# vt-asaplab/porla

Measured on NVIDIA B200. Metric: G1 MSM points/sec, higher is better.
Workload: dtype u32 (8x32-bit limb Montgomery, IMAD carry chains)

## Files before the change

### porla_b200/csrc/affine_kernels.cuh

```cuda
#pragma once
#include "msm_kernels.cuh"

namespace porla {

constexpr int kAffL = 64;
constexpr int kAffCap1 = 44;
constexpr int kAffCap2 = 24;
constexpr int kAffMaxAdds = 32;
constexpr int kAffThreads = 128;
constexpr int kAffDefaultRounds = 0;
#ifndef PORLA_AFF_MIN_BLOCKS
#define PORLA_AFF_MIN_BLOCKS 3
#endif

enum : uint32_t { kOpCopy = 0, kOpAdd = 1, kOpDbl = 2, kOpInf = 3 };

template <class C>
struct AffSrc {
    using F = typename C::F;
    const Affine<F>* points;
    const F* phi_x;
    uint32_t phi_off;
    const uint2* pairs;
    const Affine<F>* arr;
    const uint32_t* keys;

    PORLA_D uint32_t key(int i) const { return pairs ? __ldg(&pairs[i].x) : keys[i]; }
    PORLA_D Affine<F> pt(int i) const {
        if (pairs) return load_signed_point<C>(points, phi_x, phi_off, __ldg(&pairs[i].y));
        return arr[i];
    }
    PORLA_D F ptx(int i) const {
        if (pairs) {
            const uint32_t idx = __ldg(&pairs[i].y) & 0x7fffffffu;
            const bool image = C::kGlv && phi_off != 0 && idx >= phi_off;
            const uint32_t j = image ? idx - phi_off : idx;
            const uint4* sx = image ? reinterpret_cast<const uint4*>(phi_x + j) : reinterpret_cast<const uint4*>(points + j);
            F x;
            uint4* d = reinterpret_cast<uint4*>(&x);
            d[0] = __ldg(sx);
            d[1] = __ldg(sx + 1);
            return x;
        }
        return arr[i].x;
    }
};

template <class C>
PORLA_D int aff_count_outputs(const AffSrc<C>& src, int n) {
    int outs = 0, i = 0;
    while (i < n) {
        const uint32_t k = src.key(i);
        i += (i + 1 < n && src.key(i + 1) == k) ? 2 : 1;
        outs++;
    }
    return outs;
}

template <class C>
PORLA_D int aff_round(const AffSrc<C>& src, int n, uint64_t in_inf, Affine<typename C::F>* out, uint32_t* out_keys,
                      typename C::F* pre, uint8_t* opi, uint64_t* out_inf) {
    using F = typename C::F;
    int i = 0, j = 0, na = 0;
    F acc = F::one();
    while (i < n) {
        const uint32_t k = src.key(i);
        const bool pair = i + 1 < n && src.key(i + 1) == k;
        uint32_t type = kOpCopy, idx = (uint32_t)i;
        if (pair) {
            const bool inf0 = (in_inf >> i) & 1u, inf1 = (in_inf >> (i + 1)) & 1u;
            if (inf0 || inf1) {
                if (inf0 && inf1) type = kOpInf;
                else idx = (uint32_t)(inf0 ? i + 1 : i);
            } else {
                F den = src.ptx(i + 1) - src.ptx(i);
                type = kOpAdd;
                if (den.is_zero()) {
                    const Affine<F> p = src.pt(i), q = src.pt(i + 1);
                    if (p.y == q.y && !p.y.is_zero()) {
                        den = p.y.dbl();
                        type = kOpDbl;
                    } else {
                        type = kOpInf;
                    }
                }
                if (type != kOpInf) {
                    pre[na++] = acc;
                    acc = acc * den;
                }
            }
        } else if ((in_inf >> i) & 1u) {
            type = kOpInf;
        }
        opi[j] = (uint8_t)(idx | (type << 6));
        out_keys[j] = k;
        i += pair ? 2 : 1;
        j++;
    }
    const int outs = j;
    F inv = F::one();
    if (na > 0) inv = acc.inverse();
    uint64_t infm = 0;
    for (j = outs - 1; j >= 0; j--) {
        const uint32_t idx = opi[j] & 63u, type = opi[j] >> 6;
        if (type == kOpCopy) {
            out[j] = src.pt((int)idx);
        } else if (type == kOpInf) {
            infm |= 1ull << j;
        } else {
            const Affine<F> p = src.pt((int)idx), q = src.pt((int)idx + 1);
            const F den = type == kOpAdd ? q.x - p.x : p.y.dbl();
            const F inv_j = inv * pre[--na];
            inv = inv * den;
            F lam, x3;
            if (type == kOpAdd) {
                lam = (q.y - p.y) * inv_j;
                x3 = lam.sqr() - p.x - q.x;
            } else {
                const F xx = p.x.sqr();
                lam = (xx.dbl() + xx) * inv_j;
                x3 = lam.sqr() - p.x.dbl();
            }
            Affine<F> r;
            r.x = x3;
            r.y = lam * (p.x - x3) - p.y;
            out[j] = r;
        }
    }
    *out_inf = infm;
    return outs;
}

template <class C>
__global__ void __launch_bounds__(kAffThreads, PORLA_AFF_MIN_BLOCKS)
k_accumulate_affine(const Affine<typename C::F>* __restrict__ points, const typename C::F* __restrict__ phi_x, uint32_t phi_off,
                    const uint2* __restrict__ sorted, const uint32_t* __restrict__ total_pairs,
                    XYZZ<typename C::F>* __restrict__ buckets, XYZZ<typename C::F>* __restrict__ part_head,
                    XYZZ<typename C::F>* __restrict__ part_tail, int rounds) {
    using F = typename C::F;
    const uint32_t M = *total_pairs;
    const uint32_t t = blockIdx.x * blockDim.x + threadIdx.x;
    const uint64_t start64 = (uint64_t)t * kAffL;
    if (start64 >= M) return;
    const uint32_t start = (uint32_t)start64;
    const uint32_t end = (M - start > (uint32_t)kAffL) ? start + kAffL : M;
    const uint32_t prev_key = start > 0 ? __ldg(&sorted[start - 1].x) : 0xffffffffu;
    const uint32_t next_key = end < M ? __ldg(&sorted[end].x) : 0xffffffffu;

    Affine<F> p1[kAffCap1], p2[kAffCap2];
    F pre[kAffMaxAdds];
    uint32_t k1[kAffCap1], k2[kAffCap2];
    uint8_t opi[kAffCap1];

    AffSrc<C> cur;
    cur.points = points;
    cur.phi_x = phi_x;
    cur.phi_off = phi_off;
    cur.pairs = sorted + start;
    cur.arr = nullptr;
    cur.keys = nullptr;
    int n = (int)(end - start);
    uint64_t inf = 0;

    if (rounds >= 1) {
        const int outs0 = aff_count_outputs<C>(cur, n);
        if (outs0 <= kAffCap1 && outs0 < n) {
            n = aff_round<C>(cur, n, inf, p1, k1, pre, opi, &inf);
            cur.pairs = nullptr;
            cur.arr = p1;
            cur.keys = k1;
            if (rounds >= 2) {
                const int outs1 = aff_count_outputs<C>(cur, n);
                if (outs1 <= kAffCap2 && outs1 < n) {
                    n = aff_round<C>(cur, n, inf, p2, k2, pre, opi, &inf);
                    cur.arr = p2;
                    cur.keys = k2;
                }
            }
        }
    }

    int i = 0;
    while (i < n) {
        const uint32_t key = cur.key(i);
        const bool first_run = i == 0;
        XYZZ<F> acc = XYZZ<F>::inf();
        if (!((inf >> i) & 1u)) {
            const Affine<F> p = cur.pt(i);
            acc = XYZZ<F>{p.x, p.y, F::one(), F::one()};
        }
        i++;
        while (i < n && cur.key(i) == key) {
            if (!((inf >> i) & 1u)) acc.madd(cur.pt(i));
            i++;
        }
        const bool last_run = i == n;
        if (first_run && prev_key == key) st16(part_head + t, acc);
        else if (last_run && next_key == key) st16(part_tail + t, acc);
        else st16(buckets + key, acc);
    }
}

}
```

### porla_b200/csrc/msm_impl.cuh

```cuda
#pragma once
#include <atomic>
#include <cstdio>
#include <cstdlib>
#include <mutex>
#include <type_traits>

#include "arena.h"
#include "msm.h"
#include "msm_kernels.cuh"
#include "small_kernels.cuh"
#include "affine_kernels.cuh"

namespace porla {

extern std::atomic<uint64_t> g_launches;
#define LAUNCHED() (g_launches.fetch_add(1, std::memory_order_relaxed))



template <class C> struct CurveIdOf;
template <> struct CurveIdOf<Bn254> { static constexpr int value = kCurveBn254; };
template <> struct CurveIdOf<Secp256k1> { static constexpr int value = kCurveSecp256k1; };

template <class C>
// ... 161 lines not shown
    sh.c = wplan.c;
    sh.nwin = glv ? 2 * wplan.nwin : (C::kScalarBits + 1 + sh.c - 1) / sh.c;
    int slice_shift = 0;
    while ((1 << slice_shift) < opt.slice_count) slice_shift++;
    if (opt.slice_count > 1) {
        const bool ok = (1 << slice_shift) == opt.slice_count && opt.slice_index >= 0 && opt.slice_index < opt.slice_count &&
                        !fixed && nbatch == 1 && opt.window_bits > 0 && opt.glv >= 0 && opt.no_fixed_base &&
                        msm_max_slices(wplan, opt.slice_count) == opt.slice_count;
        if (!ok) {
            fprintf(stderr, "[libmultiexp/porla_b200] FATAL: bucket slice %d of %d: needs one MSM, a forced window layout and a power-of-two "
                            "slice count that leaves whole coarse bins (c = %d)\n", opt.slice_index, opt.slice_count, wplan.c);
            abort();
        }
    }
    sh.slice_shift = (uint32_t)slice_shift;
    sh.slice_r = opt.slice_count > 1 ? (uint32_t)opt.slice_index : 0u;
    sh.nbuckets = (1u << (sh.c - 1)) >> slice_shift;
    sh.fixed_n = fixed ? table.fb_n : 0u;
    sh.glv_wh = glv ? wplan.nwin : 0;
    sh.phi_off = glv ? table.phi_off : 0u;
    const int slot_windows = fixed ? 1 : (glv ? wplan.nwin : sh.nwin);

    const uint64_t slots = (uint64_t)nbatch * slot_windows;
    const uint64_t nbt64 = slots * sh.nbuckets;
    const uint64_t pairs64 = (uint64_t)nbatch * n * sh.nwin;
    if (nbt64 >= (1ull << 32) || pairs64 >= (1ull << 32) || (uint64_t)nbatch * n >= (1ull << 31) ||
        (fixed && (uint64_t)table.fb_n * sh.nwin >= (1ull << 31))) {
        fprintf(stderr, "[libmultiexp/porla_b200] FATAL: MSM shape too large for 32-bit indexing\n");
        abort();
    }
    const uint32_t nbt = (uint32_t)nbt64;
    const uint32_t ntiles = (nbt + kScanTile - 1) / kScanTile;

    uint32_t chunk = 64;
    while (chunk > 4 && (uint64_t)nbt / chunk < 24576ull) chunk >>= 1;
    while (chunk > 4 && sh.nbuckets / chunk < 4) chunk >>= 1;
    if (const char* e = getenv("PORLA_REDUCE_CHUNK")) { if (atoi(e) >= 1) chunk = (uint32_t)atoi(e); }
    if (chunk > sh.nbuckets) chunk = sh.nbuckets;
    uint32_t threads_per_slot = (sh.nbuckets + chunk - 1) / chunk;
    uint32_t blocks_per_slot = (threads_per_slot + kRedThreads - 1) / kRedThreads;
    static const uint64_t quad_max = [] { const char* e = getenv("PORLA_REDUCE_QUAD_MAX"); return e ? (uint64_t)atoll(e) : (uint64_t)C::kReduceQuadMax; }();
    static const uint64_t quad_target = [] { const char* e = getenv("PORLA_REDUCE_QUADS"); return e && atoll(e) > 0 ? (uint64_t)atoll(e) : 148ull * kQuadsPerBlock; }();
    const bool reduce_v1 = getenv("PORLA_REDUCE_V1") != nullptr || (uint64_t)nbt > quad_max;
    uint32_t log_m = 0;
    while (log_m < 6 && ((uint64_t)nbt >> log_m) > quad_target) log_m++;
    while ((sh.nbuckets >> log_m) > (uint32_t)(kTopMaxBlocks * kQuadsPerBlock)) log_m++;
    while (log_m > 0 && (1u << log_m) > sh.nbuckets) log_m--;
    const uint32_t scan_tps = sh.nbuckets >> log_m;
    const uint32_t scan_group = scan_tps >= (uint32_t)kQuadsPerBlock ? (uint32_t)kQuadsPerBlock : scan_tps;
    const uint32_t scan_bps = scan_tps >= (uint32_t)kQuadsPerBlock ? scan_tps / kQuadsPerBlock : 1u;
    if (!reduce_v1) blocks_per_slot = 2 * scan_bps;

    const uint64_t pairs_cap = pairs64 ? pairs64 : 1;
    const uint64_t pairs_geo = (pairs_cap >> slice_shift) ? (pairs_cap >> slice_shift) : 1;
    const uint64_t wave = 148ull * 4ull * kAccThreads;
    const uint64_t waves = (pairs_geo + wave * 64 - 1) / (wave * 64);
    uint32_t L = (uint32_t)((pairs_geo + waves * wave - 1) / (waves * wave));
    if (waves == 1) {
        const uint64_t l2 = pairs_geo / (wave * 18 / 25);
        if (l2 >= 16 && l2 <= 64) L = (uint32_t)l2;
    }
    if (L < 16) L = 16;
    if (L > 64) L = 64;
    if (const char* e = getenv("PORLA_SLICE_LEN")) { if (atoi(e) >= 2) L = (uint32_t)atoi(e); }
    int aff_rounds = 0;
    {
        const char* e = getenv("PORLA_ACC_AFFINE");
        const bool big = pairs_cap >= (uint64_t)148 * PORLA_AFF_MIN_BLOCKS * kAffThreads * kAffL * 2;
        const int want = e ? atoi(e) : (big ? kAffDefaultRounds : 0);
        if (want > 0 && !streamed && slice_shift == 0) {
            aff_rounds = want > 2 ? 2 : want;
            L = kAffL;
        }
    }
    const uint32_t nslices_cap = (uint32_t)((pairs_cap + L - 1) / L);
    const uint32_t serial_limit = (nslices_cap >> slice_shift) < 200000u ? kStitchSerialSmall : kStitchSerial;
    const uint32_t long_cap = (uint32_t)(pairs_cap / ((uint64_t)L * serial_limit)) + 2;

    const bool radix = nbatch == 1 && n >= (1u << 19) && sh.nwin <= 28 && sh.c >= 9 && sh.c <= 20 && (sh.nbuckets >> (sh.c / 2)) <= (uint32_t)kPartMaxBins && !getenv("PORLA_ATOMIC_SCATTER");
    const int lb = sh.c / 2;
    const uint32_t ncoarse = radix ? (nbt >> lb) : 0u;
    DeviceCtx& cx = device_ctx();
    Arena& g_arena = cx.arena;
    StageTimer& g_stage_timer = cx.timer;
    std::lock_guard<std::mutex> lock(cx.engine_mu);
    size_t need = (radix ? Arena::padded(pairs_cap, 8) + Arena::padded(ncoarse, 4) : 0) + Arena::padded(nbt, 4) * 2 + Arena::padded(ntiles + 1, 4) + 512 +
                  Arena::padded(pairs_cap, 8) + (streamed ? 0 : Arena::padded(nbt, sizeof(XYZZ<F>))) +
                  2 * Arena::padded(nslices_cap, sizeof(XYZZ<F>)) + Arena::padded(long_cap, 8) +
                  Arena::padded(slots * blocks_per_slot, sizeof(XYZZ<F>)) + Arena::padded(slots, sizeof(XYZZ<F>));
    g_arena.acquire(stream);
    g_arena.reserve(need, stream);
    g_arena.reset();
    uint32_t* counters = g_arena.take<uint32_t>(nbt);
    uint32_t* offsets = g_arena.take<uint32_t>(nbt);
    uint32_t* tile_sums = g_arena.take<uint32_t>(ntiles + 1);
    uint32_t* grand = g_arena.take<uint32_t>(1);
    uint32_t* long_count = g_arena.take<uint32_t>(1);
    uint2* sorted = g_arena.take<uint2>(pairs_cap);
    uint2* part = radix ? g_arena.take<uint2>(pairs_cap) : nullptr;
    uint32_t* coarse_cursor = radix ? g_arena.take<uint32_t>(ncoarse) : nullptr;
    XYZZ<F>* buckets = streamed ? reinterpret_cast<XYZZ<F>*>(opt.d_buckets) : g_arena.take<XYZZ<F>>(nbt);
    const int into = opt.part_mode == kPartMiddle || opt.part_mode == kPartLast;
    XYZZ<F>* part_head = g_arena.take<XYZZ<F>>(nslices_cap);
    XYZZ<F>* part_tail = g_arena.take<XYZZ<F>>(nslices_cap);
    uint2* long_runs = g_arena.take<uint2>(long_cap);
    XYZZ<F>* partials = g_arena.take<XYZZ<F>>(slots * blocks_per_slot);
    XYZZ<F>* wsum = g_arena.take<XYZZ<F>>(slots);

    const Affine<F>* points = reinterpret_cast<const Affine<F>*>(fixed ? table.d_fb_points : table.d_points);
    using FC = typename C::FC;
    using XC = XYZZ<FC>;
    static_assert(sizeof(XC) == sizeof(XYZZ<F>), "layouts must coincide");
    const uint64_t total_scalars = (uint64_t)n * nbatch;

    g_stage_timer.mark(kStageCount, stream);
    const char* sv2 = getenv("PORLA_SORT_V2");
    const bool v2_fits = ncoarse > 0 && pairs_cap / ncoarse <= (uint64_t)(kBigBin * 0.95);
    const bool sort_v2 = radix && slice_shift == 0 && lb <= 10 && (size_t)ncoarse * 4 <= (160u << 10) && (sv2 ? sv2[0] == '1' : v2_fits);
    PORLA_CUDA(cudaMemsetAsync(counters, 0, (size_t)nbt * 4, stream));
    PORLA_CUDA(cudaMemsetAsync(grand, 0, 4, stream));
    PORLA_CUDA(cudaMemsetAsync(long_count, 0, 4, stream));
    static_assert(sizeof(XYZZ<F>) == 128, "k_fine_smem / k_big_scan clear 128-byte bucket records");
    if (!into && !sort_v2) PORLA_CUDA(cudaMemsetAsync(buckets, 0, (size_t)nbt * sizeof(XYZZ<F>), stream));
    uint4* zero_buckets = into ? nullptr : reinterpret_cast<uint4*>(buckets);
    if (total_scalars && sort_v2) {
        static std::once_flag attr_once_dev2[kMaxDevices];
        const size_t smem0 = (size_t)ncoarse * 4;
        const size_t smem1 = ((size_t)9 * kPartTile + 2 * kPartMaxBins) * 4 + (size_t)kPartTile * 8;
        const size_t smem2 = (size_t)2 * kFineHist * 4 + (size_t)kFineTile * 8;
        const size_t smem3 = (size_t)kBigBin * 6 + (size_t)kFineLocalBuckets * 4;
        std::call_once(attr_once_dev2[current_device()], [=] {
            PORLA_CUDA(cudaFuncSetAttribute(k_coarse_count<C, false>, cudaFuncAttributeMaxDynamicSharedMemorySize, 160 << 10));
            PORLA_CUDA(cudaFuncSetAttribute(k_partition_coarse<C, false>, cudaFuncAttributeMaxDynamicSharedMemorySize, (int)smem1));
            if constexpr (C::kGlv) {
                PORLA_CUDA(cudaFuncSetAttribute(k_coarse_count<C, true>, cudaFuncAttributeMaxDynamicSharedMemorySize, 160 << 10));
                PORLA_CUDA(cudaFuncSetAttribute(k_partition_coarse<C, true>, cudaFuncAttributeMaxDynamicSharedMemorySize, (int)smem1));
            }
            PORLA_CUDA(cudaFuncSetAttribute(k_partition_fine_big, cudaFuncAttributeMaxDynamicSharedMemorySize, (int)smem2));
            PORLA_CUDA(cudaFuncSetAttribute(k_fine_smem, cudaFuncAttributeMaxDynamicSharedMemorySize, (int)smem3));
        });
        uint32_t* coarse_count = offsets;
        uint32_t* coarse_off = offsets + ncoarse + 1;
        PORLA_CUDA(cudaMemsetAsync(coarse_count, 0, (size_t)(ncoarse + 1) * 4, stream));
        uint32_t cgrid = (uint32_t)((total_scalars + kCoarseCountThreads - 1) / kCoarseCountThreads);
        if (cgrid > 148u * 2u) cgrid = 148u * 2u;
        bool glv_done = false;
        if constexpr (C::kGlv) {
            if (glv) {
                k_coarse_count<C, true><<<cgrid, kCoarseCountThreads, smem0, stream>>>(d_scalars, opt.scalar_be, table.d_flags, sh, lb, ncoarse, coarse_count);
                glv_done = true;
            }
        }
        if (!glv_done)
            k_coarse_count<C, false><<<cgrid, kCoarseCountThreads, smem0, stream>>>(d_scalars, opt.scalar_be, table.d_flags, sh, lb, ncoarse, coarse_count);
        LAUNCHED();
        g_stage_timer.mark(kStageScan, stream);
        k_coarse_scan<<<1, 1024, 0, stream>>>(coarse_count, ncoarse, coarse_off, coarse_cursor, grand);
        LAUNCHED();
        g_stage_timer.mark(kStageScatter, stream);
        glv_done = false;
// ... 41 lines not shown
        if (radix) {
            static std::once_flag attr_once_dev[kMaxDevices];
            std::once_flag& attr_once = attr_once_dev[current_device()];
            const size_t smem1 = ((size_t)9 * kPartTile + 2 * kPartMaxBins) * 4 + (size_t)kPartTile * 8;
            const size_t smem2 = (size_t)2 * kFineHist * 4 + (size_t)kFineTile * 8;
            std::call_once(attr_once, [=] {
                PORLA_CUDA(cudaFuncSetAttribute(k_partition_coarse<C, false>, cudaFuncAttributeMaxDynamicSharedMemorySize, (int)smem1));
                if constexpr (C::kGlv)
                    PORLA_CUDA(cudaFuncSetAttribute(k_partition_coarse<C, true>, cudaFuncAttributeMaxDynamicSharedMemorySize, (int)smem1));
                PORLA_CUDA(cudaFuncSetAttribute(k_partition_fine, cudaFuncAttributeMaxDynamicSharedMemorySize, (int)smem2));
            });
            k_init_coarse<<<(ncoarse + 255) / 256, 256, 0, stream>>>(offsets, nbt, lb, ncoarse, coarse_cursor);
            LAUNCHED();
            bool coarse_glv = false;
            if constexpr (C::kGlv) {
                if (glv) {
                    k_partition_coarse<C, true><<<(n + kPartTile - 1) / kPartTile, kPartThreads, smem1, stream>>>(
                        d_scalars, opt.scalar_be, table.d_flags, sh, lb, coarse_cursor, part);
                    coarse_glv = true;
                }
            }
            if (!coarse_glv)
                k_partition_coarse<C, false><<<(n + kPartTile - 1) / kPartTile, kPartThreads, smem1, stream>>>(
                    d_scalars, opt.scalar_be, table.d_flags, sh, lb, coarse_cursor, part);
            LAUNCHED();
            k_partition_fine<<<(uint32_t)((pairs_cap + kFineTile - 1) / kFineTile), kFineThreads, smem2, stream>>>(part, grand, lb,
                                                                                                             counters, sorted);
            LAUNCHED();
        } else {
        int wgroup = sh.nwin;
        if (nbatch == 1) {
            uint64_t per_window = (uint64_t)n * 8;
            wgroup = (int)((64ull << 20) / (per_window ? per_window : 1));
            if (wgroup < 1) wgroup = 1;
            if (wgroup > sh.nwin) wgroup = sh.nwin;
        }
        for (int w0 = 0; w0 < sh.nwin; w0 += wgroup) {
            int w1 = w0 + wgroup < sh.nwin ? w0 + wgroup : sh.nwin;
            bool scatter_glv = false;
            if constexpr (C::kGlv) {
                if (glv) {
                    k_digits<C, true, true><<<grid, 256, 0, stream>>>(d_scalars, opt.scalar_be, table.d_flags, sh, w0, w1, counters, sorted);
                    scatter_glv = true;
                }
            }
            if (!scatter_glv)
                k_digits<C, true, false><<<grid, 256, 0, stream>>>(d_scalars, opt.scalar_be, table.d_flags, sh, w0, w1, counters, sorted);
            LAUNCHED();
        }
        }
    }
    if (total_scalars) {
        g_stage_timer.mark(kStageAccumulate, stream);
        if (aff_rounds > 0)
            k_accumulate_affine<C><<<(nslices_cap + kAffThreads - 1) / kAffThreads, kAffThreads, 0, stream>>>(
                points, reinterpret_cast<const F*>(table.d_phi_x), sh.phi_off, sorted, grand, buckets, part_head, part_tail, aff_rounds);
        else
            k_accumulate<C><<<(nslices_cap + kAccThreads - 1) / kAccThreads, kAccThreads, 0, stream>>>(
                points, reinterpret_cast<const F*>(table.d_phi_x), sh.phi_off, sorted, grand, L, buckets, part_head, part_tail, into);
        LAUNCHED();
        if (getenv("PORLA_STITCH_COMPACT"))
            k_stitch<C, FC><<<(nslices_cap + 63) / 64, 64, 0, stream>>>(sorted, grand, L, (XC*)buckets, (const XC*)part_head,
                                                                       (const XC*)part_tail, long_count, long_runs, serial_limit);
        else
            k_stitch<C, F><<<(nslices_cap + 63) / 64, 64, 0, stream>>>(sorted, grand, L, buckets, part_head, part_tail,
                                                                      long_count, long_runs, serial_limit);
        LAUNCHED();
        k_stitch_long<C><<<148, kLongThreads, 0, stream>>>(sorted, grand, L, (XC*)buckets, (const XC*)part_head, long_count,
                                                          long_runs);
        LAUNCHED();
    } else {
        g_stage_timer.mark(kStageScan, stream);
        g_stage_timer.mark(kStageScatter, stream);
        g_stage_timer.mark(kStageAccumulate, stream);
    }
    g_stage_timer.mark(kStageReduce, stream);
    if (opt.part_mode == kPartFirst || opt.part_mode == kPartMiddle) {
        g_stage_timer.mark(kStageFinalize, stream);
        g_stage_timer.mark(kNumStages, stream);
        g_arena.release(stream);
        PORLA_CUDA(cudaGetLastError());
        return;
    }
    if (slots * blocks_per_slot >= (1ull << 31)) {
        fprintf(stderr, "[libmultiexp/porla_b200] FATAL: too many window slots for one launch\n");
        abort();
    }
    const XYZZ<F>* window_sums = partials;
    if (reduce_v1) {
        const uint32_t rgrid = threads_per_slot >= (uint32_t)kRedThreads
                                   ? (uint32_t)(slots * blocks_per_slot)
                                   : (uint32_t)((slots + kRedThreads / threads_per_slot - 1) / (kRedThreads / threads_per_slot));
        k_reduce<C><<<rgrid, kRedThreads, 0, stream>>>((const XC*)buckets, sh.nbuckets, chunk, threads_per_slot, (uint32_t)slots,
                                                       (XC*)partials, sh.slice_shift, sh.slice_r);
        LAUNCHED();
        if (blocks_per_slot > 1) {
            k_window_sums<C><<<(uint32_t)slots, kRedThreads, 0, stream>>>((const XC*)partials, blocks_per_slot, (XC*)wsum);
            LAUNCHED();
            window_sums = wsum;
        }
    } else {
        XYZZ<F>* out_w = partials;
        XYZZ<F>* out_s = out_w + slots * scan_bps;
        const uint32_t sgrid = scan_group == (uint32_t)kQuadsPerBlock
                                   ? (uint32_t)(slots * scan_bps)
                                   : (uint32_t)((slots + kQuadsPerBlock / scan_group - 1) / (kQuadsPerBlock / scan_group));
        k_reduce_scan<C><<<sgrid, kQuadThreads, 0, stream>>>(buckets, sh.nbuckets, log_m, scan_group, (uint32_t)slots, out_w, out_s);
        LAUNCHED();
        if (scan_bps > 1 || sh.slice_shift != 0) {
            uint32_t log_u = log_m;
            while ((1u << log_u) < ((uint32_t)kQuadsPerBlock << log_m)) log_u++;
            k_reduce_top<C><<<(uint32_t)slots, kQuadThreads, 0, stream>>>(out_w, out_s, scan_bps, log_u, sh.slice_shift, sh.slice_r, wsum);
            LAUNCHED();
            window_sums = wsum;
        }
    }
    g_stage_timer.mark(kStageFinalize, stream);
    if (opt.d_window_sums) {
        PORLA_CUDA(cudaMemcpyAsync(opt.d_window_sums, window_sums, slots * sizeof(XYZZ<F>), cudaMemcpyDeviceToDevice, stream));
    } else {
        k_finalize<C><<<(nbatch + 31) / 32, 32, 0, stream>>>((const XC*)window_sums, nbatch, slot_windows, sh.c, opt.out_fmt, d_out,
                                                            reinterpret_cast<XC*>(d_out_xyzz));
        LAUNCHED();
    }
    g_stage_timer.mark(kNumStages, stream);
    g_arena.release(stream);
    PORLA_CUDA(cudaGetLastError());
// ... 152 lines not shown
```

### porla_b200/csrc/msm_kernels.cuh

```cuda
#pragma once
#include "ec.cuh"
#include "quad.cuh"

namespace porla {

enum ScalarFormat : int { kScalarBE32 = 0, kScalarLE32 = 1 };
enum PointFormat : int { kPointBE64 = 0, kPointLE64 = 1 };

struct MsmShape {
    uint32_t n;
    uint32_t nbatch;
    uint32_t shared;
    int c;
    int nwin;
    uint32_t nbuckets;
    uint32_t fixed_n;
    int glv_wh;
    uint32_t phi_off;
    uint32_t slice_shift;
    uint32_t slice_r;
};

PORLA_D uint32_t slice_bucket(const MsmShape& sh, uint32_t mag) {
    const uint32_t b = mag - 1u;
// ... 892 lines not shown
    }
    __syncthreads();
#pragma unroll
    for (int q = 0; q < kFinePerThread; q++) {
        if (e[q].x == 0xffffffffu) continue;
        const uint32_t rel = e[q].x - kbase;
        if (rel < kFineHist) stage[cnt[rel] + rank[q]] = e[q];
        else sorted[atomicAdd(&cursor[e[q].x], 1u)] = e[q];
    }
    __syncthreads();
    const uint32_t total = s_total;
    for (uint32_t j = threadIdx.x; j < total; j += kFineThreads) {
        const uint2 x = stage[j];
        sorted[delta[x.x - kbase] + j] = x;
    }
}

constexpr int kAccThreads = 128;
#ifndef PORLA_ACC_MIN_BLOCKS
#define PORLA_ACC_MIN_BLOCKS 4
#endif

template <class C>
PORLA_D Affine<typename C::F> load_signed_point(const Affine<typename C::F>* __restrict__ points,
                                                const typename C::F* __restrict__ phi_x, uint32_t phi_off, uint32_t e) {
    using F = typename C::F;
    const uint32_t idx = e & 0x7fffffffu;
    const bool image = C::kGlv && phi_off != 0 && idx >= phi_off;
    const uint32_t j = image ? idx - phi_off : idx;
    const uint4* sx = image ? reinterpret_cast<const uint4*>(phi_x + j) : reinterpret_cast<const uint4*>(points + j);
    const uint4* sy = reinterpret_cast<const uint4*>(points + j) + 2;
    Affine<F> p;
    uint4* d = reinterpret_cast<uint4*>(&p);
    d[0] = __ldg(sx);
    d[1] = __ldg(sx + 1);
    d[2] = __ldg(sy);
    d[3] = __ldg(sy + 1);
    if (e >> 31) p.y = p.y.neg();
    return p;
}

template <class F>
PORLA_D XYZZ<F> bucket_seed(const XYZZ<F>* __restrict__ buckets, uint32_t key, int into) {
    XYZZ<F> acc = XYZZ<F>::inf();
    if (into) {
        const uint4* s = reinterpret_cast<const uint4*>(buckets + key);
        uint4* d = reinterpret_cast<uint4*>(&acc);
#pragma unroll
        for (int i = 0; i < 8; i++) d[i] = s[i];
    }
    return acc;
}

template <class C>
__global__ void __launch_bounds__(kAccThreads, PORLA_ACC_MIN_BLOCKS)
k_accumulate(const Affine<typename C::F>* __restrict__ points, const typename C::F* __restrict__ phi_x, uint32_t phi_off,
             const uint2* __restrict__ sorted, const uint32_t* __restrict__ total_pairs, uint32_t L,
             XYZZ<typename C::F>* __restrict__ buckets, XYZZ<typename C::F>* __restrict__ part_head,
             XYZZ<typename C::F>* __restrict__ part_tail, int into) {
    using F = typename C::F;
    const uint32_t M = *total_pairs;
    const uint32_t t = blockIdx.x * blockDim.x + threadIdx.x;
    const uint64_t start64 = (uint64_t)t * L;
    if (start64 >= M) return;
    const uint32_t start = (uint32_t)start64;
    const uint32_t end = (M - start > L) ? start + L : M;
    const uint32_t prev_key = start > 0 ? __ldg(&sorted[start - 1].x) : 0xffffffffu;
    const uint32_t next_key = end < M ? __ldg(&sorted[end].x) : 0xffffffffu;

    uint32_t key = __ldg(&sorted[start].x);
    bool first = true;
    XYZZ<F> acc = prev_key == key ? XYZZ<F>::inf() : bucket_seed<F>(buckets, key, into);
    for (uint32_t pos = start; pos < end; ++pos) {
        const uint2 e = __ldg(&sorted[pos]);
        const Affine<F> q = load_signed_point<C>(points, phi_x, phi_off, e.y);
        if (e.x != key) {
            if (first && prev_key == key) st16(part_head + t, acc);
            else st16(buckets + key, acc);
            first = false;
            key = e.x;
            acc = bucket_seed<F>(buckets, key, into);
        }
        if (acc.is_inf()) acc = XYZZ<F>{q.x, q.y, F::one(), F::one()};
        else acc.madd_finite(q);
    }
    if (first && prev_key == key) st16(part_head + t, acc);
    else if (next_key == key) st16(part_tail + t, acc);
    else st16(buckets + key, acc);
}

constexpr uint32_t kStitchSerial = 48;
constexpr uint32_t kStitchSerialSmall = 8;

template <class C, class F>
__global__ void __launch_bounds__(64)
k_stitch(const uint2* __restrict__ sorted, const uint32_t* __restrict__ total_pairs, uint32_t L,
         XYZZ<F>* __restrict__ buckets, const XYZZ<F>* __restrict__ part_head,
         const XYZZ<F>* __restrict__ part_tail, uint32_t* __restrict__ long_count,
         uint2* __restrict__ long_runs, uint32_t serial_limit) {
    const uint32_t M = *total_pairs;
    const uint32_t t = blockIdx.x * blockDim.x + threadIdx.x;
    const uint64_t start64 = (uint64_t)t * L;
    if (start64 >= M) return;
    const uint32_t start = (uint32_t)start64;
    if (M - start <= L) return;
    const uint32_t end = start + L;
    const uint32_t key = __ldg(&sorted[end - 1].x);
    if (__ldg(&sorted[end].x) != key) return;
    if (__ldg(&sorted[start].x) == key && start > 0 && __ldg(&sorted[start - 1].x) == key) return;
    const uint32_t nslices = (uint32_t)(((uint64_t)M + L - 1) / L);
    uint32_t u = t + 1, cnt = 0;
    XYZZ<F> acc = ld16(part_tail + t);
    for (;;) {
        if (cnt == serial_limit) {
            st16(buckets + key, acc);
            uint32_t slot = atomicAdd(long_count, 1u);
            long_runs[slot] = make_uint2(key, u);
            return;
        }
        acc.add(ld16(part_head + u));
        cnt++;
        uint32_t uend = (u + 1 < nslices) ? (u + 1) * L : M;
        if (u + 1 < nslices && __ldg(&sorted[uend - 1].x) == key && __ldg(&sorted[uend].x) == key) u++;
        else break;
    }
    st16(buckets + key, acc);
}

constexpr int kLongThreads = 128;

template <class C>
__global__ void __launch_bounds__(kLongThreads)
k_stitch_long(const uint2* __restrict__ sorted, const uint32_t* __restrict__ total_pairs, uint32_t L,
              XYZZ<typename C::FC>* __restrict__ buckets, const XYZZ<typename C::FC>* __restrict__ part_head,
              const uint32_t* __restrict__ long_count, const uint2* __restrict__ long_runs) {
    using F = typename C::FC;
    __shared__ XYZZ<F> sh[kLongThreads];
    __shared__ uint32_t s_last;
    const uint32_t M = *total_pairs;
    const uint32_t nruns = *long_count;
    const uint32_t nslices = (uint32_t)(((uint64_t)M + L - 1) / L);
    for (uint32_t r = blockIdx.x; r < nruns; r += gridDim.x) {
        const uint32_t key = long_runs[r].x, u0 = long_runs[r].y;
        if (threadIdx.x == 0) {
            uint32_t lo = u0 * L, hi = M;
            while (hi - lo > 1) {
                uint32_t mid = lo + (hi - lo) / 2;
                if (__ldg(&sorted[mid].x) == key) lo = mid;
                else hi = mid;
            }
            s_last = lo / L;
        }
        __syncthreads();
        const uint32_t last = s_last < nslices ? s_last : nslices - 1;
        XYZZ<F> acc = XYZZ<F>::inf();
        for (uint32_t u = u0 + threadIdx.x; u <= last; u += kLongThreads) acc.add(ld16(part_head + u));
        sh[threadIdx.x] = acc;
        __syncthreads();
        for (int o = kLongThreads / 2; o > 0; o >>= 1) {
            if ((int)threadIdx.x < o) {
                XYZZ<F> a = sh[threadIdx.x];
                a.add(sh[threadIdx.x + o]);
// ... 771 lines not shown
```

Before: 309.8 million.

## Add multi-kernel batched-affine bucket reduction rounds and in-kernel cut stitching

Swaps the per-thread affine pairing kernel for a grid-wide scheme. Run-bounds and per-round output offsets are computed first, then each round does a forward pass of prefix products, a block-level product tree, one inversion per block and a finish pass that writes the halved affine point lists. k_accumulate also gains ticket-based stitching, so a thread that completes the second half of a two-slice cut merges the partial sums itself and k_stitch skips those single cuts. The affine rounds are opt-in through PORLA_ACC_AFFINE, but the ticket stitching and the cut_ticket memset appear to apply on the default path. This adds atomics and threadfences per cut in exchange for fewer serial stitch steps.

```diff
diff --git a/porla_b200/csrc/affine_kernels.cuh b/porla_b200/csrc/affine_kernels.cuh
--- a/porla_b200/csrc/affine_kernels.cuh
+++ b/porla_b200/csrc/affine_kernels.cuh
@@ -3,202 +3,214 @@
 
 namespace porla {
 
-constexpr int kAffL = 64;
-constexpr int kAffCap1 = 44;
-constexpr int kAffCap2 = 24;
-constexpr int kAffMaxAdds = 32;
-constexpr int kAffThreads = 128;
-constexpr int kAffDefaultRounds = 0;
-#ifndef PORLA_AFF_MIN_BLOCKS
-#define PORLA_AFF_MIN_BLOCKS 3
+constexpr int kRoundThreads = 128;
+#ifndef PORLA_ROUND_K
+#define PORLA_ROUND_K 16
 #endif
-
-enum : uint32_t { kOpCopy = 0, kOpAdd = 1, kOpDbl = 2, kOpInf = 3 };
+constexpr int kRoundK = PORLA_ROUND_K;
+constexpr int kRoundMinBlocks = 4;
+constexpr uint32_t kRoundBatch = kRoundThreads * kRoundK;
+constexpr int kMaxAffineRounds = 6;
+
+static __global__ void __launch_bounds__(256)
+k_run_bounds(const uint2* __restrict__ pairs, const uint32_t* __restrict__ total, uint32_t* __restrict__ start,
+             uint32_t* __restrict__ end) {
+    const uint32_t M = *total;
+    for (uint32_t i = blockIdx.x * blockDim.x + threadIdx.x; i < M; i += gridDim.x * blockDim.x) {
+        const uint32_t key = __ldg(&pairs[i].x);
+        if (i == 0 || __ldg(&pairs[i - 1].x) != key) start[key] = i;
+        if (i + 1 == M || __ldg(&pairs[i + 1].x) != key) end[key] = i + 1;
+    }
+}
+
+static __global__ void __launch_bounds__(256)
+k_round_counts(const uint32_t* __restrict__ start, const uint32_t* __restrict__ end, uint32_t nbt, int r,
+               uint32_t* __restrict__ cnt) {
+    const uint32_t b = blockIdx.x * blockDim.x + threadIdx.x;
+    if (b >= nbt) return;
+    const uint32_t m = end[b] - start[b];
+    cnt[b] = (uint32_t)(((uint64_t)m + (1u << r) - 1) >> r);
+}
+
+template <class C, bool kPairs>
+PORLA_D Affine<typename C::F> round_input(const Affine<typename C::F>* __restrict__ points, const typename C::F* __restrict__ phi_x,
+                                          uint32_t phi_off, const uint2* __restrict__ pairs,
+                                          const Affine<typename C::F>* __restrict__ in, uint32_t i) {
+    if constexpr (kPairs) return load_signed_point<C>(points, phi_x, phi_off, __ldg(&pairs[i].y));
+    else return ld16(in + i);
+}
+
+template <class F>
+PORLA_D F pair_den(const Affine<F>& p, const Affine<F>& q, bool& add, bool& dbl) {
+    const bool live = !p.is_inf() && !q.is_inf();
+    const F dx = q.x - p.x;
+    const bool same_x = dx.is_zero();
+    add = live && !same_x;
+    dbl = live && same_x && q.y == p.y;
+    return add ? dx : (dbl ? p.y.dbl() : F::one());
+}
 
 template <class C>
-struct AffSrc {
+struct RoundIo {
     using F = typename C::F;
     const Affine<F>* points;
     const F* phi_x;
     uint32_t phi_off;
     const uint2* pairs;
-    const Affine<F>* arr;
-    const uint32_t* keys;
-
-    PORLA_D uint32_t key(int i) const { return pairs ? __ldg(&pairs[i].x) : keys[i]; }
-    PORLA_D Affine<F> pt(int i) const {
-        if (pairs) return load_signed_point<C>(points, phi_x, phi_off, __ldg(&pairs[i].y));
-        return arr[i];
-    }
-    PORLA_D F ptx(int i) const {
-        if (pairs) {
-            const uint32_t idx = __ldg(&pairs[i].y) & 0x7fffffffu;
-            const bool image = C::kGlv && phi_off != 0 && idx >= phi_off;
-            const uint32_t j = image ? idx - phi_off : idx;
-            const uint4* sx = image ? reinterpret_cast<const uint4*>(phi_x + j) : reinterpret_cast<const uint4*>(points + j);
-            F x;
-            uint4* d = reinterpret_cast<uint4*>(&x);
-            d[0] = __ldg(sx);
-            d[1] = __ldg(sx + 1);
-            return x;
-        }
-        return arr[i].x;
-    }
+    const Affine<F>* in;
+    const uint32_t* in_start;
+    const uint32_t* in_end;
+    const uint32_t* out_off;
+    uint32_t nbt;
 };
 
+PORLA_D uint32_t round_bucket(const uint32_t* __restrict__ out_off, uint32_t nbt, uint32_t j) {
+    uint32_t lo = 0, hi = nbt;
+    while (hi - lo > 1) {
+        const uint32_t mid = lo + (hi - lo) / 2;
+        if (__ldg(&out_off[mid]) <= j) lo = mid;
+        else hi = mid;
+    }
+    return lo;
+}
+
+struct RoundCursor {
+    uint32_t b, lo, hi, in0, in1;
+
+    template <class C>
+    PORLA_D void seek(const RoundIo<C>& io, uint32_t j) {
+        if (j >= lo && j < hi) return;
+        if (j >= hi) {
+            do b++;
+            while (__ldg(&io.out_off[b + 1]) <= j);
+        } else {
+            do b--;
+            while (__ldg(&io.out_off[b]) > j);
+        }
+        load(io);
+    }
+    template <class C>
+    PORLA_D void load(const RoundIo<C>& io) {
+        lo = __ldg(&io.out_off[b]);
+        hi = __ldg(&io.out_off[b + 1]);
+        in0 = __ldg(&io.in_start[b]);
+        in1 = __ldg(&io.in_end[b]);
+    }
+};
+
+template <class C, bool kPairs>
+PORLA_D void round_operands(const RoundIo<C>& io, RoundCursor& cur, uint32_t j, bool valid, Affine<typename C::F>& p,
+                            Affine<typename C::F>& q) {
+    p = Affine<typename C::F>::inf();
+    q = Affine<typename C::F>::inf();
+    if (!valid) return;
+    cur.seek(io, j);
+    const uint32_t a = cur.in0 + 2 * (j - cur.lo);
+    p = round_input<C, kPairs>(io.points, io.phi_x, io.phi_off, io.pairs, io.in, a);
+    if (a + 1 < cur.in1) q = round_input<C, kPairs>(io.points, io.phi_x, io.phi_off, io.pairs, io.in, a + 1);
+}
+
+template <class C, bool kPairs>
+__global__ void __launch_bounds__(kRoundThreads, kRoundMinBlocks)
+k_round_forward(RoundIo<C> io, typename C::F* __restrict__ pre, typename C::F* __restrict__ tree) {
+    using F = typename C::F;
+    __shared__ F sh[2 * kRoundThreads];
+    const uint32_t M = __ldg(&io.out_off[io.nbt]);
+    const uint32_t t = threadIdx.x;
+    if ((uint64_t)blockIdx.x * kRoundBatch >= M) return;
+    const uint32_t j0 = (blockIdx.x * kRoundThreads + t) * kRoundK;
+    F* bpre = pre + (size_t)blockIdx.x * kRoundBatch;
+    RoundCursor cur{j0 < M ? round_bucket(io.out_off, io.nbt, j0) : 0u};
+    if (j0 < M) cur.load(io);
+    F acc = F::one();
+#pragma unroll 4
+    for (int k = 0; k < kRoundK; k++) {
+        const uint32_t j = j0 + k;
+        Affine<F> p, q;
+        round_operands<C, kPairs>(io, cur, j, j < M, p, q);
+        bool add, dbl;
+        const F den = pair_den(p, q, add, dbl);
+        st16(bpre + k * kRoundThreads + t, acc);
+        acc = acc * den;
+    }
+    sh[kRoundThreads + t] = acc;
+    __syncthreads();
+#pragma unroll 1
+    for (uint32_t s = kRoundThreads / 2; s >= 1; s >>= 1) {
+        if (t < s) sh[s + t] = sh[2 * (s + t)] * sh[2 * (s + t) + 1];
+        __syncthreads();
+    }
+    F* btree = tree + (size_t)blockIdx.x * 2 * kRoundThreads;
+    st16(btree + kRoundThreads + t, sh[kRoundThreads + t]);
+    if (t) st16(btree + t, sh[t]);
+}
+
 template <class C>
-PORLA_D int aff_count_outputs(const AffSrc<C>& src, int n) {
-    int outs = 0, i = 0;
-    while (i < n) {
-        const uint32_t k = src.key(i);
-        i += (i + 1 < n && src.key(i + 1) == k) ? 2 : 1;
-        outs++;
-    }
-    return outs;
-}
-
-template <class C>
-PORLA_D int aff_round(const AffSrc<C>& src, int n, uint64_t in_inf, Affine<typename C::F>* out, uint32_t* out_keys,
-                      typename C::F* pre, uint8_t* opi, uint64_t* out_inf) {
+__global__ void __launch_bounds__(64)
+k_round_invert(const uint32_t* __restrict__ out_off, uint32_t nbt, uint32_t nblocks, typename C::F* __restrict__ tree) {
+    const uint32_t i = blockIdx.x * blockDim.x + threadIdx.x;
+    if (i >= nblocks || (uint64_t)i * kRoundBatch >= __ldg(&out_off[nbt])) return;
+    typename C::F* root = tree + (size_t)i * 2 * kRoundThreads + 1;
+    st16(root, ld16(root).inverse());
+}
+
+template <class C, bool kPairs>
+__global__ void __launch_bounds__(kRoundThreads, kRoundMinBlocks)
+k_round_finish(RoundIo<C> io, const typename C::F* __restrict__ pre, const typename C::F* __restrict__ tree,
+               Affine<typename C::F>* __restrict__ out, uint2* __restrict__ out_keys) {
     using F = typename C::F;
-    int i = 0, j = 0, na = 0;
-    F acc = F::one();
-    while (i < n) {
-        const uint32_t k = src.key(i);
-        const bool pair = i + 1 < n && src.key(i + 1) == k;
-        uint32_t type = kOpCopy, idx = (uint32_t)i;
-        if (pair) {
-            const bool inf0 = (in_inf >> i) & 1u, inf1 = (in_inf >> (i + 1)) & 1u;
-            if (inf0 || inf1) {
-                if (inf0 && inf1) type = kOpInf;
-                else idx = (uint32_t)(inf0 ? i + 1 : i);
-            } else {
-                F den = src.ptx(i + 1) - src.ptx(i);
-                type = kOpAdd;
-                if (den.is_zero()) {
-                    const Affine<F> p = src.pt(i), q = src.pt(i + 1);
-                    if (p.y == q.y && !p.y.is_zero()) {
-                        den = p.y.dbl();
-                        type = kOpDbl;
-                    } else {
-                        type = kOpInf;
-                    }
-                }
-                if (type != kOpInf) {
-                    pre[na++] = acc;
-                    acc = acc * den;
-                }
-            }
-        } else if ((in_inf >> i) & 1u) {
-            type = kOpInf;
-        }
-        opi[j] = (uint8_t)(idx | (type << 6));
-        out_keys[j] = k;
-        i += pair ? 2 : 1;
-        j++;
-    }
-    const int outs = j;
-    F inv = F::one();
-    if (na > 0) inv = acc.inverse();
-    uint64_t infm = 0;
-    for (j = outs - 1; j >= 0; j--) {
-        const uint32_t idx = opi[j] & 63u, type = opi[j] >> 6;
-        if (type == kOpCopy) {
-            out[j] = src.pt((int)idx);
-        } else if (type == kOpInf) {
-            infm |= 1ull << j;
-        } else {
-            const Affine<F> p = src.pt((int)idx), q = src.pt((int)idx + 1);
-            const F den = type == kOpAdd ? q.x - p.x : p.y.dbl();
-            const F inv_j = inv * pre[--na];
-            inv = inv * den;
-            F lam, x3;
-            if (type == kOpAdd) {
-                lam = (q.y - p.y) * inv_j;
-                x3 = lam.sqr() - p.x - q.x;
-            } else {
-                const F xx = p.x.sqr();
-                lam = (xx.dbl() + xx) * inv_j;
-                x3 = lam.sqr() - p.x.dbl();
-            }
-            Affine<F> r;
-            r.x = x3;
-            r.y = lam * (p.x - x3) - p.y;
-            out[j] = r;
-        }
-    }
-    *out_inf = infm;
-    return outs;
-}
-
-template <class C>
-__global__ void __launch_bounds__(kAffThreads, PORLA_AFF_MIN_BLOCKS)
-k_accumulate_affine(const Affine<typename C::F>* __restrict__ points, const typename C::F* __restrict__ phi_x, uint32_t phi_off,
-                    const uint2* __restrict__ sorted, const uint32_t* __restrict__ total_pairs,
-                    XYZZ<typename C::F>* __restrict__ buckets, XYZZ<typename C::F>* __restrict__ part_head,
-                    XYZZ<typename C::F>* __restrict__ part_tail, int rounds) {
-    using F = typename C::F;
-    const uint32_t M = *total_pairs;
-    const uint32_t t = blockIdx.x * blockDim.x + threadIdx.x;
-    const uint64_t start64 = (uint64_t)t * kAffL;
-    if (start64 >= M) return;
-    const uint32_t start = (uint32_t)start64;
-    const uint32_t end = (M - start > (uint32_t)kAffL) ? start + kAffL : M;
-    const uint32_t prev_key = start > 0 ? __ldg(&sorted[start - 1].x) : 0xffffffffu;
-    const uint32_t next_key = end < M ? __ldg(&sorted[end].x) : 0xffffffffu;
-
-    Affine<F> p1[kAffCap1], p2[kAffCap2];
-    F pre[kAffMaxAdds];
-    uint32_t k1[kAffCap1], k2[kAffCap2];
-    uint8_t opi[kAffCap1];
-
-    AffSrc<C> cur;
-    cur.points = points;
-    cur.phi_x = phi_x;
-    cur.phi_off = phi_off;
-    cur.pairs = sorted + start;
-    cur.arr = nullptr;
-    cur.keys = nullptr;
-    int n = (int)(end - start);
-    uint64_t inf = 0;
-
-    if (rounds >= 1) {
-        const int outs0 = aff_count_outputs<C>(cur, n);
-        if (outs0 <= kAffCap1 && outs0 < n) {
-            n = aff_round<C>(cur, n, inf, p1, k1, pre, opi, &inf);
-            cur.pairs = nullptr;
-            cur.arr = p1;
-            cur.keys = k1;
-            if (rounds >= 2) {
-                const int outs1 = aff_count_outputs<C>(cur, n);
-                if (outs1 <= kAffCap2 && outs1 < n) {
-                    n = aff_round<C>(cur, n, inf, p2, k2, pre, opi, &inf);
-                    cur.arr = p2;
-                    cur.keys = k2;
-                }
-            }
-        }
-    }
-
-    int i = 0;
-    while (i < n) {
-        const uint32_t key = cur.key(i);
-        const bool first_run = i == 0;
-        XYZZ<F> acc = XYZZ<F>::inf();
-        if (!((inf >> i) & 1u)) {
-            const Affine<F> p = cur.pt(i);
-            acc = XYZZ<F>{p.x, p.y, F::one(), F::one()};
-        }
-        i++;
-        while (i < n && cur.key(i) == key) {
-            if (!((inf >> i) & 1u)) acc.madd(cur.pt(i));
-            i++;
-        }
-        const bool last_run = i == n;
-        if (first_run && prev_key == key) st16(part_head + t, acc);
-        else if (last_run && next_key == key) st16(part_tail + t, acc);
-        else st16(buckets + key, acc);
-    }
-}
-
-}
+    __shared__ F sh[2 * kRoundThreads];
+    const uint32_t M = __ldg(&io.out_off[io.nbt]);
+    const uint32_t t = threadIdx.x;
+    if ((uint64_t)blockIdx.x * kRoundBatch >= M) return;
+    const F* btree = tree + (size_t)blockIdx.x * 2 * kRoundThreads;
+    sh[kRoundThreads + t] = ld16(btree + kRoundThreads + t);
+    if (t) sh[t] = ld16(btree + t);
+    __syncthreads();
+#pragma unroll 1
+    for (uint32_t s = 1; s < (uint32_t)kRoundThreads; s <<= 1) {
+        if (t < s) {
+            const uint32_t v = s + t;
+            const F inv = sh[v], l = sh[2 * v], r = sh[2 * v + 1];
+            sh[2 * v] = inv * r;
+            sh[2 * v + 1] = inv * l;
+        }
+        __syncthreads();
+    }
+    F inv = sh[kRoundThreads + t];
+    const F* bpre = pre + (size_t)blockIdx.x * kRoundBatch;
+    const uint32_t j0 = (blockIdx.x * kRoundThreads + t) * kRoundK;
+    RoundCursor cur{j0 < M ? round_bucket(io.out_off, io.nbt, (M - j0 > (uint32_t)kRoundK ? j0 + kRoundK : M) - 1) : 0u};
+    if (j0 < M) cur.load(io);
+    Affine<F> pn, qn;
+    round_operands<C, kPairs>(io, cur, j0 + kRoundK - 1, j0 + kRoundK - 1 < M, pn, qn);
+#pragma unroll 1
+    for (int k = kRoundK - 1; k >= 0; k--) {
+        const uint32_t j = j0 + k;
+        const bool valid = j < M;
+        const uint32_t b = cur.b;
+        const Affine<F> p = pn, q = qn;
+        if (k) round_operands<C, kPairs>(io, cur, j - 1, j - 1 < M, pn, qn);
+        bool add, dbl;
+        const F den = pair_den(p, q, add, dbl);
+        const F inv_k = inv * ld16(bpre + k * kRoundThreads + t);
+        if (k) inv = inv * den;
+        F num = q.y - p.y;
+        if (__any_sync(0xffffffffu, dbl)) {
+            const F xx = p.x.sqr();
+            const F tri = xx.dbl() + xx;
+            if (dbl) num = tri;
+        }
+        const F lam = num * inv_k;
+        Affine<F> r;
+        r.x = lam.sqr() - p.x - q.x;
+        r.y = lam * (p.x - r.x) - p.y;
+        if (!(add || dbl)) r = p.is_inf() ? q : (q.is_inf() ? p : Affine<F>::inf());
+        if (valid) {
+            st16(out + j, r);
+            if (out_keys) out_keys[j] = make_uint2(b, j);
+        }
+    }
+}
+
+}
diff --git a/porla_b200/csrc/msm_impl.cuh b/porla_b200/csrc/msm_impl.cuh
--- a/porla_b200/csrc/msm_impl.cuh
+++ b/porla_b200/csrc/msm_impl.cuh
@@ -237,7 +237,22 @@
     if (!reduce_v1) blocks_per_slot = 2 * scan_bps;
 
     const uint64_t pairs_cap = pairs64 ? pairs64 : 1;
-    const uint64_t pairs_geo = (pairs_cap >> slice_shift) ? (pairs_cap >> slice_shift) : 1;
+    int aff_rounds = 0;
+    uint64_t aff_bound[kMaxAffineRounds + 1] = {pairs_cap};
+    if (!streamed && slice_shift == 0 && nbatch == 1) {
+        if (const char* e = getenv("PORLA_ACC_AFFINE")) {
+            const int want = atoi(e);
+            aff_rounds = want < 0 ? 0 : (want > kMaxAffineRounds ? kMaxAffineRounds : want);
+        }
+        for (int r = 0; r < aff_rounds; r++) {
+            const uint64_t half = (aff_bound[r] + 1) / 2 + nbt;
+            aff_bound[r + 1] = half < aff_bound[r] ? half : aff_bound[r];
+        }
+        if (aff_rounds > 0 && aff_bound[1] >= (1ull << 31)) aff_rounds = 0;
+    }
+    const uint64_t acc_cap = aff_bound[aff_rounds];
+    uint64_t pairs_geo = (acc_cap >> slice_shift) ? (acc_cap >> slice_shift) : 1;
+    if (aff_rounds > 0 && (pairs_cap >> aff_rounds) + nbt / 2 < pairs_geo) pairs_geo = (pairs_cap >> aff_rounds) + nbt / 2;
     const uint64_t wave = 148ull * 4ull * kAccThreads;
     const uint64_t waves = (pairs_geo + wave * 64 - 1) / (wave * 64);
     uint32_t L = (uint32_t)((pairs_geo + waves * wave - 1) / (waves * wave));
@@ -248,19 +263,9 @@
     if (L < 16) L = 16;
     if (L > 64) L = 64;
     if (const char* e = getenv("PORLA_SLICE_LEN")) { if (atoi(e) >= 2) L = (uint32_t)atoi(e); }
-    int aff_rounds = 0;
-    {
-        const char* e = getenv("PORLA_ACC_AFFINE");
-        const bool big = pairs_cap >= (uint64_t)148 * PORLA_AFF_MIN_BLOCKS * kAffThreads * kAffL * 2;
-        const int want = e ? atoi(e) : (big ? kAffDefaultRounds : 0);
-        if (want > 0 && !streamed && slice_shift == 0) {
-            aff_rounds = want > 2 ? 2 : want;
-            L = kAffL;
-        }
-    }
-    const uint32_t nslices_cap = (uint32_t)((pairs_cap + L - 1) / L);
+    const uint32_t nslices_cap = (uint32_t)((acc_cap + L - 1) / L);
     const uint32_t serial_limit = (nslices_cap >> slice_shift) < 200000u ? kStitchSerialSmall : kStitchSerial;
-    const uint32_t long_cap = (uint32_t)(pairs_cap / ((uint64_t)L * serial_limit)) + 2;
+    const uint32_t long_cap = (uint32_t)(acc_cap / ((uint64_t)L * serial_limit)) + 2;
 
     const bool radix = nbatch == 1 && n >= (1u << 19) && sh.nwin <= 28 && sh.c >= 9 && sh.c <= 20 && (sh.nbuckets >> (sh.c / 2)) <= (uint32_t)kPartMaxBins && !getenv("PORLA_ATOMIC_SCATTER");
     const int lb = sh.c / 2;
@@ -271,8 +276,14 @@
     std::lock_guard<std::mutex> lock(cx.engine_mu);
     size_t need = (radix ? Arena::padded(pairs_cap, 8) + Arena::padded(ncoarse, 4) : 0) + Arena::padded(nbt, 4) * 2 + Arena::padded(ntiles + 1, 4) + 512 +
                   Arena::padded(pairs_cap, 8) + (streamed ? 0 : Arena::padded(nbt, sizeof(XYZZ<F>))) +
-                  2 * Arena::padded(nslices_cap, sizeof(XYZZ<F>)) + Arena::padded(long_cap, 8) +
+                  2 * Arena::padded(nslices_cap, sizeof(XYZZ<F>)) + Arena::padded(nslices_cap, 4) + Arena::padded(long_cap, 8) +
                   Arena::padded(slots * blocks_per_slot, sizeof(XYZZ<F>)) + Arena::padded(slots, sizeof(XYZZ<F>));
+    const uint64_t round_blocks = (aff_bound[1] + kRoundBatch - 1) / kRoundBatch;
+    if (aff_rounds > 0)
+        need += 2 * Arena::padded(nbt, 4) + aff_rounds * Arena::padded((size_t)nbt + 1, 4) +
+                Arena::padded(aff_bound[1], sizeof(Affine<F>)) + (aff_rounds > 1 ? Arena::padded(aff_bound[2], sizeof(Affine<F>)) : 0) +
+                Arena::padded(acc_cap, 8) + Arena::padded(round_blocks * kRoundBatch, sizeof(F)) +
+                Arena::padded(round_blocks * 2 * kRoundThreads, sizeof(F));
     g_arena.acquire(stream);
     g_arena.reserve(need, stream);
     g_arena.reset();
@@ -288,9 +299,27 @@
     const int into = opt.part_mode == kPartMiddle || opt.part_mode == kPartLast;
     XYZZ<F>* part_head = g_arena.take<XYZZ<F>>(nslices_cap);
     XYZZ<F>* part_tail = g_arena.take<XYZZ<F>>(nslices_cap);
+    uint32_t* cut_ticket = g_arena.take<uint32_t>(nslices_cap);
     uint2* long_runs = g_arena.take<uint2>(long_cap);
     XYZZ<F>* partials = g_arena.take<XYZZ<F>>(slots * blocks_per_slot);
     XYZZ<F>* wsum = g_arena.take<XYZZ<F>>(slots);
+    uint32_t* run_start = nullptr;
+    uint32_t* run_end = nullptr;
+    uint32_t* round_off[kMaxAffineRounds + 1] = {};
+    Affine<F>* round_buf[2] = {};
+    uint2* round_keys = nullptr;
+    F* round_pre = nullptr;
+    F* round_tree = nullptr;
+    if (aff_rounds > 0) {
+        round_pre = g_arena.take<F>(round_blocks * kRoundBatch);
+        round_tree = g_arena.take<F>(round_blocks * 2 * kRoundThreads);
+        run_start = g_arena.take<uint32_t>(nbt);
+        run_end = g_arena.take<uint32_t>(nbt);
+        for (int r = 1; r <= aff_rounds; r++) round_off[r] = g_arena.take<uint32_t>((size_t)nbt + 1);
+        round_buf[0] = g_arena.take<Affine<F>>(aff_bound[1]);
+        if (aff_rounds > 1) round_buf[1] = g_arena.take<Affine<F>>(aff_bound[2]);
+        round_keys = g_arena.take<uint2>(acc_cap);
+    }
 
     const Affine<F>* points = reinterpret_cast<const Affine<F>*>(fixed ? table.d_fb_points : table.d_points);
     using FC = typename C::FC;
@@ -438,27 +467,67 @@
     }
     if (total_scalars) {
         g_stage_timer.mark(kStageAccumulate, stream);
-        if (aff_rounds > 0)
-            k_accumulate_affine<C><<<(nslices_cap + kAffThreads - 1) / kAffThreads, kAffThreads, 0, stream>>>(
-                points, reinterpret_cast<const F*>(table.d_phi_x), sh.phi_off, sorted, grand, buckets, part_head, part_tail, aff_rounds);
+        PORLA_CUDA(cudaMemsetAsync(cut_ticket, 0, (size_t)nslices_cap * 4, stream));
+        const uint2* acc_list = sorted;
+        const uint32_t* acc_total = grand;
+        if (aff_rounds > 0) {
+            PORLA_CUDA(cudaMemsetAsync(run_start, 0, (size_t)nbt * 4, stream));
+            PORLA_CUDA(cudaMemsetAsync(run_end, 0, (size_t)nbt * 4, stream));
+            uint32_t bgrid = (uint32_t)((pairs_cap + 255) / 256);
+            if (bgrid > 148u * 16u) bgrid = 148u * 16u;
+            k_run_bounds<<<bgrid, 256, 0, stream>>>(sorted, grand, run_start, run_end);
+            LAUNCHED();
+            for (int r = 1; r <= aff_rounds; r++) {
+                k_round_counts<<<(nbt + 255) / 256, 256, 0, stream>>>(run_start, run_end, nbt, r, offsets);
+                LAUNCHED();
+                k_scan_tiles<<<ntiles, kScanThreads, 0, stream>>>(offsets, round_off[r], nbt, tile_sums);
+                LAUNCHED();
+                k_scan_sums<<<1, kScanThreads, 0, stream>>>(tile_sums, ntiles, round_off[r] + nbt);
+                LAUNCHED();
+                k_scan_add<<<ntiles, kScanThreads, 0, stream>>>(round_off[r], counters, nbt, tile_sums);
+                LAUNCHED();
+            }
+            for (int r = 0; r < aff_rounds; r++) {
+                const uint32_t grid = (uint32_t)((aff_bound[r + 1] + kRoundBatch - 1) / kRoundBatch);
+                RoundIo<C> io{points, reinterpret_cast<const F*>(table.d_phi_x), sh.phi_off, sorted, nullptr, run_start, run_end,
+                              round_off[r + 1], nbt};
+                if (r > 0) io = RoundIo<C>{nullptr, nullptr, 0u, nullptr, round_buf[(r - 1) & 1], round_off[r], round_off[r] + 1,
+                                           round_off[r + 1], nbt};
+                Affine<F>* out = round_buf[r & 1];
+                uint2* keys = r + 1 == aff_rounds ? round_keys : nullptr;
+                if (r == 0) k_round_forward<C, true><<<grid, kRoundThreads, 0, stream>>>(io, round_pre, round_tree);
+                else k_round_forward<C, false><<<grid, kRoundThreads, 0, stream>>>(io, round_pre, round_tree);
+                LAUNCHED();
+                k_round_invert<C><<<(grid + 63) / 64, 64, 0, stream>>>(round_off[r + 1], nbt, grid, round_tree);
+                LAUNCHED();
+                if (r == 0) k_round_finish<C, true><<<grid, kRoundThreads, 0, stream>>>(io, round_pre, round_tree, out, keys);
+                else k_round_finish<C, false><<<grid, kRoundThreads, 0, stream>>>(io, round_pre, round_tree, out, keys);
+                LAUNCHED();
+            }
+            acc_list = round_keys;
+            acc_total = round_off[aff_rounds] + nbt;
+            k_accumulate<C, true><<<(nslices_cap + kAccThreads - 1) / kAccThreads, kAccThreads, 0, stream>>>(
+                round_buf[(aff_rounds - 1) & 1], nullptr, 0u, acc_list, acc_total, L, buckets, part_head, part_tail, 0, cut_ticket);
+        } else {
+            k_accumulate<C><<<(nslices_cap + kAccThreads - 1) / kAccThreads, kAccThreads, 0, stream>>>(
+                points, reinterpret_cast<const F*>(table.d_phi_x), sh.phi_off, sorted, grand, L, buckets, part_head, part_tail, into, cut_ticket);
+        }
+        LAUNCHED();
+        if (getenv("PORLA_STITCH_COMPACT"))
+            k_stitch<C, FC><<<(nslices_cap + 63) / 64, 64, 0, stream>>>(acc_list, acc_total, L, (XC*)buckets, (const XC*)part_head,
+                                                                       (const XC*)part_tail, long_count, long_runs, serial_limit, 1);
         else
-            k_accumulate<C><<<(nslices_cap + kAccThreads - 1) / kAccThreads, kAccThreads, 0, stream>>>(
-                points, reinterpret_cast<const F*>(table.d_phi_x), sh.phi_off, sorted, grand, L, buckets, part_head, part_tail, into);
-        LAUNCHED();
-        if (getenv("PORLA_STITCH_COMPACT"))
-            k_stitch<C, FC><<<(nslices_cap + 63) / 64, 64, 0, stream>>>(sorted, grand, L, (XC*)buckets, (const XC*)part_head,
-                                                                       (const XC*)part_tail, long_count, long_runs, serial_limit);
-        else
-            k_stitch<C, F><<<(nslices_cap + 63) / 64, 64, 0, stream>>>(sorted, grand, L, buckets, part_head, part_tail,
-                                                                      long_count, long_runs, serial_limit);
-        LAUNCHED();
-        k_stitch_long<C><<<148, kLongThreads, 0, stream>>>(sorted, grand, L, (XC*)buckets, (const XC*)part_head, long_count,
+            k_stitch<C, F><<<(nslices_cap + 63) / 64, 64, 0, stream>>>(acc_list, acc_total, L, buckets, part_head, part_tail,
+                                                                      long_count, long_runs, serial_limit, 1);
+        LAUNCHED();
+        k_stitch_long<C><<<148, kLongThreads, 0, stream>>>(acc_list, acc_total, L, (XC*)buckets, (const XC*)part_head, long_count,
                                                           long_runs);
         LAUNCHED();
     } else {
         g_stage_timer.mark(kStageScan, stream);
         g_stage_timer.mark(kStageScatter, stream);
         g_stage_timer.mark(kStageAccumulate, stream);
+        PORLA_CUDA(cudaMemsetAsync(cut_ticket, 0, (size_t)nslices_cap * 4, stream));
     }
     g_stage_timer.mark(kStageReduce, stream);
     if (opt.part_mode == kPartFirst || opt.part_mode == kPartMiddle) {
diff --git a/porla_b200/csrc/msm_kernels.cuh b/porla_b200/csrc/msm_kernels.cuh
--- a/porla_b200/csrc/msm_kernels.cuh
+++ b/porla_b200/csrc/msm_kernels.cuh
@@ -968,12 +968,12 @@
     return acc;
 }
 
-template <class C>
+template <class C, bool kRecords = false>
 __global__ void __launch_bounds__(kAccThreads, PORLA_ACC_MIN_BLOCKS)
 k_accumulate(const Affine<typename C::F>* __restrict__ points, const typename C::F* __restrict__ phi_x, uint32_t phi_off,
              const uint2* __restrict__ sorted, const uint32_t* __restrict__ total_pairs, uint32_t L,
              XYZZ<typename C::F>* __restrict__ buckets, XYZZ<typename C::F>* __restrict__ part_head,
-             XYZZ<typename C::F>* __restrict__ part_tail, int into) {
+             XYZZ<typename C::F>* __restrict__ part_tail, int into, uint32_t* __restrict__ ticket) {
     using F = typename C::F;
     const uint32_t M = *total_pairs;
     const uint32_t t = blockIdx.x * blockDim.x + threadIdx.x;
@@ -985,6 +985,7 @@
     const uint32_t next_key = end < M ? __ldg(&sorted[end].x) : 0xffffffffu;
 
     uint32_t key = __ldg(&sorted[start].x);
+    const uint32_t key0 = key;
     bool first = true;
     XYZZ<F> acc = prev_key == key ? XYZZ<F>::inf() : bucket_seed<F>(buckets, key, into);
     for (uint32_t pos = start; pos < end; ++pos) {
@@ -997,12 +998,50 @@
             key = e.x;
             acc = bucket_seed<F>(buckets, key, into);
         }
+        if (kRecords && q.is_inf()) continue;
         if (acc.is_inf()) acc = XYZZ<F>{q.x, q.y, F::one(), F::one()};
         else acc.madd_finite(q);
     }
+    const bool tail = !(first && prev_key == key) && next_key == key;
     if (first && prev_key == key) st16(part_head + t, acc);
-    else if (next_key == key) st16(part_tail + t, acc);
+    else if (tail) st16(part_tail + t, acc);
     else st16(buckets + key, acc);
+    if (!ticket) return;
+#pragma unroll 1
+    for (int s = 0; s < 2; s++) {
+        uint32_t u, k;
+        if (s == 0) {
+            if (prev_key != key0) continue;
+            if (first && next_key == key0) continue;
+            const uint32_t ustart = start - L;
+            if (__ldg(&sorted[ustart].x) == key0 && ustart > 0 && __ldg(&sorted[ustart - 1].x) == key0) continue;
+            u = t - 1;
+            k = key0;
+        } else {
+            if (!tail) continue;
+            const uint32_t e2 = M - end > L ? end + L : M;
+            if (e2 < M && __ldg(&sorted[e2].x) == key) continue;
+            u = t;
+            k = key;
+        }
+        __threadfence();
+        if (atomicAdd(ticket + u, 1u) != 1u) continue;
+        __threadfence();
+        const XYZZ<F>* mine = s == 0 ? part_head + t : part_tail + t;
+        const XYZZ<F>* other = s == 0 ? part_tail + u : part_head + u + 1;
+        XYZZ<typename C::FC> a, b;
+        const uint4* sa = reinterpret_cast<const uint4*>(mine);
+        const uint4* sb = reinterpret_cast<const uint4*>(other);
+        uint4* da = reinterpret_cast<uint4*>(&a);
+        uint4* db = reinterpret_cast<uint4*>(&b);
+#pragma unroll
+        for (int i = 0; i < 8; i++) {
+            da[i] = __ldcg(sa + i);
+            db[i] = __ldcg(sb + i);
+        }
+        a.add(b);
+        st16(reinterpret_cast<XYZZ<typename C::FC>*>(buckets + k), a);
+    }
 }
 
 constexpr uint32_t kStitchSerial = 48;
@@ -1013,7 +1052,7 @@
 k_stitch(const uint2* __restrict__ sorted, const uint32_t* __restrict__ total_pairs, uint32_t L,
          XYZZ<F>* __restrict__ buckets, const XYZZ<F>* __restrict__ part_head,
          const XYZZ<F>* __restrict__ part_tail, uint32_t* __restrict__ long_count,
-         uint2* __restrict__ long_runs, uint32_t serial_limit) {
+         uint2* __restrict__ long_runs, uint32_t serial_limit, int skip_single_cuts) {
     const uint32_t M = *total_pairs;
     const uint32_t t = blockIdx.x * blockDim.x + threadIdx.x;
     const uint64_t start64 = (uint64_t)t * L;
@@ -1024,6 +1063,10 @@
     const uint32_t key = __ldg(&sorted[end - 1].x);
     if (__ldg(&sorted[end].x) != key) return;
     if (__ldg(&sorted[start].x) == key && start > 0 && __ldg(&sorted[start - 1].x) == key) return;
+    if (skip_single_cuts) {
+        const uint32_t e2 = M - end > L ? end + L : M;
+        if (e2 == M || __ldg(&sorted[e2].x) != key) return;
+    }
     const uint32_t nslices = (uint32_t)(((uint64_t)M + L - 1) / L);
     uint32_t u = t + 1, cnt = 0;
     XYZZ<F> acc = ld16(part_tail + t);
```

After: 292.8 million (median of 6 runs). 0.945x the previous value.
